# Weepingchestnut/SAVSR

Measured on AMD Instinct MI355X. Metric: HR Mpixels/sec (Vid4-shape x4, 7-frame window), higher is better.
Workload: dtype f32 (bf16x3 split products, fp32 accumulate)

## Files before the change

### savsr_amd/csrc/conv_wy.hip

```cpp
#include "conv_common.hpp"

#include <type_traits>

#ifndef WY_STAMPS
#define WY_STAMPS 0
#endif
#ifndef WY_VALU
#define WY_VALU 6
#endif
#ifndef WY_FAST_EPILOGUE
#define WY_FAST_EPILOGUE 1
#endif
#ifndef WY_BUF
#define WY_BUF 1
#endif

namespace savsr {

namespace wy {
constexpr int TH = 16, TW = 32, NTHR = 512, COT = 64;
[[maybe_unused]] constexpr int IC = TW + 2;
#ifndef WY_ICP
#define WY_ICP 36
#endif
constexpr int ICP = WY_ICP;
constexpr int V_PLANE = 2 * ICP;
constexpr int V_WAVE = 2 * 2 * 2 * V_PLANE;
constexpr int W_HALF = 6 * 2 * 2 * 64;
constexpr int W_PHASE = 2 * W_HALF;
constexpr int EPS = 36;
constexpr int LDS_UNITS = 8 * V_WAVE + 2 * W_HALF;
constexpr size_t LDS_BYTES = 16ull * LDS_UNITS + 4ull * 8 * 32 * EPS;
static_assert(LDS_BYTES <= 160 * 1024, "LDS budget");
}

__device__ __attribute__((aligned(16))) const float g_wy_zero16[4] = {0.f, 0.f, 0.f, 0.f};

#if WY_STAMPS
__device__ long long g_wy_stamps[256 * 8 * 8];
#define WY_KSEC(i) (WY_STAMPS == 2 ? 0 : (i))
#define WY_MARK(i) do { const long long t_now = (long long)__builtin_amdgcn_s_memtime(); wy_sec[i] += t_now - wy_prev; wy_prev = t_now; } while (0)
#if WY_STAMPS == 2
#define WY_EMARK(i) WY_MARK(i)
#endif
#else
#define WY_KSEC(i) (i)
#define WY_MARK(i) do { } while (0)
#endif

__device__ __forceinline__ void wy_split_store(const f32x4& v, bf16x4* hi_dst, bf16x4* lo_dst) {
    bf16x4 hi, lo;
#pragma unroll
    for (int j = 0; j < 4; ++j) {
        const __bf16 hh = (__bf16)v[j];
        hi[j] = hh;
        lo[j] = (__bf16)(v[j] - (float)hh);
    }
    *hi_dst = hi;
    *lo_dst = lo;
}
__device__ __forceinline__ void wy_f16_store(const f32x4& v, bf16x4* hi_dst) {
    f16x4 h;
#pragma unroll
    for (int j = 0; j < 4; ++j) h[j] = (_Float16)v[j];
    *hi_dst = __builtin_bit_cast(bf16x4, h);
}

template <bool FAST, bool F16>
__global__ __launch_bounds__(512) void conv_wy_kernel(const MultiConvParams mp) {
    using namespace wy;
    constexpr int WPH = F16 ? W_PHASE / 2 : W_PHASE, WHF = F16 ? W_HALF / 2 : W_HALF;
    extern __shared__ __attribute__((aligned(16))) unsigned char smem_raw[];
    bf16x8* smem = reinterpret_cast<bf16x8*>(smem_raw);
    const int tid = threadIdx.x, lane = tid & 63, wave = tid >> 6, half = lane >> 5, px = lane & 31;
    const int wave_s = __builtin_amdgcn_readfirstlane(wave);
    const int tiles_per_cob = mp.wy_tiles;
    const int total = mp.nconv * mp.ncob * tiles_per_cob;
    const int H = mp.h, W = mp.w;

    struct TileInfo { int conv, cob, x0, y0, tx, ty, strip; };
    auto decode = [&](int tile) {
        const int cc = (int)((unsigned)tile / (unsigned)tiles_per_cob), rem = tile - cc * tiles_per_cob;
        const bool strip = rem >= mp.wy_full;
        const int tyf = (int)((unsigned)rem / (unsigned)mp.ntx);
        const int l2 = strip ? mp.wy_strip_l2 : 3;
        const int ty = strip ? mp.nty - 1 : tyf;
        const int tx = strip ? (rem - mp.wy_full) << (3 - l2) : rem - tyf * mp.ntx;
        const int wx = tx + (wave_s >> l2);
        TileInfo ti;
        ti.conv = (int)((unsigned)cc / (unsigned)mp.ncob);
        ti.cob = cc - ti.conv * mp.ncob;
        ti.x0 = (wx < mp.ntx ? wx : tx) * TW;
        ti.y0 = wx < mp.ntx ? ty * TH - 2 * ((wave_s >> l2) << l2) : mp.nty * TH;
        ti.tx = tx;
        ti.ty = ty;
        ti.strip = strip ? 1 : 0;
        return ti;
    };

    f32x4 d[2][4], dx;
#if !WY_BUF
    int st_pxb[2], st_pxt;
    constexpr int INVALID = -(1 << 30);
#endif
    const float* st_base = nullptr;
    const bf16x8* st_w = nullptr;
    int st_pix = 0, st_cb = 0, st_src = 0, st_conv = 0, st_row0 = 0;
    const int q4 = lane & 3;
#if WY_BUF
    constexpr unsigned OOB = 0x80000000u;
    unsigned st_vcol[2], st_vtail;
    int st_x0 = 0;
    auto stage_cols = [&]() {
#pragma unroll
        for (int r = 0; r < 2; ++r) {
            const int x = st_x0 - 1 + (lane >> 2) + 16 * r;
            const unsigned v = (unsigned)(x * st_pix + 4 * q4) * 4u;
            st_vcol[r] = (unsigned)x < (unsigned)W ? v : OOB;
        }
        const int x = st_x0 - 1 + 32 + ((lane & 7) >> 2), rr = (lane >> 3) & 3, row = st_row0 + rr;
        const unsigned vt = (unsigned)((rr * W + x) * st_pix + 4 * q4) * 4u;
        const bool okt = (lane < 32) & ((unsigned)x < (unsigned)W) & ((unsigned)row < (unsigned)H);
        st_vtail = okt ? vt : OOB;
    };
#endif
#if WY_BUF
    auto uni = [](int v) { return __builtin_amdgcn_readfirstlane(v); };
    auto uni_ptr = [](const float* q) {
        const unsigned long long a = (unsigned long long)(uintptr_t)q;
        const unsigned lo = (unsigned)__builtin_amdgcn_readfirstlane((int)(unsigned)a), hi = (unsigned)__builtin_amdgcn_readfirstlane((int)(unsigned)(a >> 32));
        return (const float*)(uintptr_t)(((unsigned long long)hi << 32) | lo);
    };
#else
    auto uni = [](int v) { return v; };
    auto uni_ptr = [](const float* q) { return q; };
#endif
    auto stage_begin_tile = [&](const TileInfo& ti) {
        st_conv = ti.conv;
        st_src = 0;
        st_cb = 0;
        st_base = uni_ptr(mp.c[ti.conv].src[0]);
        st_pix = uni(mp.c[ti.conv].src_pix[0]);
        st_w = reinterpret_cast<const bf16x8*>(mp.c[ti.conv].wimg) + (long long)ti.cob * mp.nchunk * WPH;
        st_row0 = uni(ti.y0 + 2 * wave_s - 1);
#if WY_BUF
        st_x0 = ti.x0;
        stage_cols();
#else
#pragma unroll
        for (int r = 0; r < 2; ++r) {
            const int x = ti.x0 - 1 + (lane >> 2) + 16 * r;
            st_pxb[r] = (x >= 0 && x < W) ? st_row0 * W + x : INVALID;
        }
        {
            const int x = ti.x0 - 1 + 32 + ((lane & 7) >> 2), row = st_row0 + ((lane >> 3) & 3);
            st_pxt = (lane < 32 && x >= 0 && x < W && row >= 0 && row < H) ? row * W + x : INVALID;
        }
#endif
    };
    auto stage_advance = [&]() {
        st_cb += 16;
        st_w += WPH;
        if (st_cb >= mp.src_ch) {
            st_cb = 0;
            ++st_src;
            st_base = uni_ptr(mp.c[st_conv].src[st_src]);
#if WY_BUF
            const int pix_new = uni(mp.c[st_conv].src_pix[st_src]);
            if (pix_new != st_pix) { st_pix = pix_new; stage_cols(); }
#else
            st_pix = mp.c[st_conv].src_pix[st_src];
#endif
        }
    };
    int st_tile = blockIdx.x, st_chunk = 0;
    auto stage_next = [&]() -> bool {
        if (st_chunk + 1 < mp.nchunk) { ++st_chunk; stage_advance(); return true; }
        if (st_tile + (int)gridDim.x >= total) return false;
        st_tile += gridDim.x;
        st_chunk = 0;
        stage_begin_tile(decode(st_tile));
        return true;
    };
#if WY_BUF
    typedef unsigned u32x4_t __attribute__((ext_vector_type(4)));
    auto row_rsrc = [&](int i, bool whole) {
        const int off = ((st_row0 + i) * W * st_pix + st_cb) * 4;
        const bool row_ok = whole || (st_row0 + i >= 0 && st_row0 + i < H);
        return __builtin_amdgcn_make_buffer_rsrc((void*)((const char*)st_base + off), (short)0, row_ok ? 0x7fffffff : 0, 0x00020000);
    };
    auto issue_row = [&](int r, int i) {
        d[r][i] = __builtin_bit_cast(f32x4, (u32x4_t)__builtin_amdgcn_raw_buffer_load_b128(row_rsrc(i, false), (int)st_vcol[r], 0, 0));
    };
    auto issue_d = [&](int r) {
#pragma unroll
        for (int i = 0; i < 4; ++i) issue_row(r, i);
    };
    auto issue_dx = [&]() { dx = __builtin_bit_cast(f32x4, (u32x4_t)__builtin_amdgcn_raw_buffer_load_b128(row_rsrc(0, true), (int)st_vtail, 0, 0)); };
#else
    auto load_at = [&](int pixel, bool ok) -> f32x4 {
        const SAVSR_GLOBAL float* src = ok ? (const SAVSR_GLOBAL float*)st_base + (pixel * st_pix + st_cb + 4 * q4)
                                           : (const SAVSR_GLOBAL float*)g_wy_zero16;
        return *(const SAVSR_GLOBAL f32x4*)src;
    };
    auto issue_row = [&](int r, int i) {
        const bool row_ok = st_row0 + i >= 0 && st_row0 + i < H;
        d[r][i] = load_at(st_pxb[r] + i * W, row_ok && st_pxb[r] != INVALID);
    };
    auto issue_d = [&](int r) {
#pragma unroll
        for (int i = 0; i < 4; ++i) issue_row(r, i);
    };
    auto issue_dx = [&]() { dx = load_at(st_pxt, st_pxt != INVALID); };
#endif
    bf16x8* vwave = smem + wave * V_WAVE;
    constexpr int PLANE_B = V_PLANE * 16;
    const unsigned vst0 = (unsigned)(wave * V_WAVE + (q4 >> 1) * ICP + (lane >> 2)) * 16u + (unsigned)(q4 & 1) * 8u;
    const unsigned vst_t = (unsigned)(wave * V_WAVE + (q4 >> 1) * ICP + 32 + ((lane & 7) >> 2)) * 16u + (unsigned)(q4 & 1) * 8u;
    auto vptr = [&](unsigned off) { return reinterpret_cast<bf16x4*>(smem_raw + off); };
    auto vstore = [&](const f32x4& v, unsigned off) {
        if constexpr (F16) wy_f16_store(v, vptr(off));
        else wy_split_store(v, vptr(off), vptr(off + PLANE_B));
    };
    auto store_pair = [&](int r, int hf, const f32x4& va, const f32x4& vb) {
        vstore(va, vst0 + (unsigned)(r * 256 + (hf * 2 + 0) * 2 * PLANE_B));
        vstore(vb, vst0 + (unsigned)(r * 256 + (hf * 2 + 1) * 2 * PLANE_B));
    };
    auto store_one = [&](int r, int hf, int vr, const f32x4& v) {
        vstore(v, vst0 + (unsigned)(r * 256 + (hf * 2 + vr) * 2 * PLANE_B));
    };
    auto store_v0 = [&](int r) { store_one(r, 0, 0, d[r][0] - d[r][2]); };
    auto store_v1 = [&](int r) {
        store_one(r, 0, 1, d[r][1] + d[r][2]);
        const f32x4 v2 = d[r][2] - d[r][1], v3 = d[r][1] - d[r][3];
        d[r][0] = v2;
        d[r][1] = v3;
    };
    auto store_v01 = [&](int r) { store_v0(r); store_v1(r); };
    auto store_v23 = [&](int r) { store_pair(r, 1, d[r][0], d[r][1]); };
    const int grp = (lane >> 3) & 3;
    auto tail_value = [&](int hf) -> f32x4 {
        const int partner = hf == 0 ? (grp == 0 ? lane ^ 16 : lane ^ 24) : (grp == 2 ? lane ^ 24 : lane ^ 16);
        f32x4 o;
#pragma unroll
        for (int j = 0; j < 4; ++j) o[j] = __shfl(dx[j], partner, 64);
        return (hf == 0 && grp == 1) ? dx + o : dx - o;
    };
    auto tail_store = [&](int hf, const f32x4& v) {
        const bool mine = lane < 32 && (hf == 0 ? grp < 2 : (grp == 2 || grp == 1));
        const int vr = hf == 0 ? grp : (grp == 2 ? 0 : 1);
        if (mine) {
            vstore(v, vst_t + (unsigned)((hf * 2 + vr) * 2 * PLANE_B));
        }
    };
    auto store_vt01 = [&]() {
        const f32x4 v01 = tail_value(0), v23 = tail_value(1);
        tail_store(0, v01);
        dx = v23;
    };
    auto store_vt23 = [&]() { tail_store(1, dx); };
    bf16x8* wlds = smem + 8 * V_WAVE;
    [[maybe_unused]] const unsigned lane16 = (unsigned)lane * 16u;
    auto issue_w = [&](int j, int hf) {
        const int piece = F16 ? j * 8 + wave_s : wave_s * 3 + j;
        if (F16 && piece >= 12) return;
        const unsigned dst = __builtin_amdgcn_readfirstlane((unsigned)(uintptr_t)(wlds + hf * W_HALF + piece * (F16 ? 128 : 64)));
        unsigned keep;
#if WY_BUF
        asm volatile("s_mov_b32 %0, m0\n\ts_mov_b32 m0, %3\n\ts_nop 0\n\tglobal_load_lds_dwordx4 %1, %2\n\ts_mov_b32 m0, %0"
                     : "=&s"(keep) : "v"(lane16), "s"(st_w + hf * WHF + piece * 64), "s"(dst) : "memory");
#else
        asm volatile("s_mov_b32 %0, m0\n\ts_mov_b32 m0, %2\n\ts_nop 0\n\tglobal_load_lds_dwordx4 %1, off\n\ts_mov_b32 m0, %0"
                     : "=&s"(keep) : "v"(st_w + hf * WHF + piece * 64 + lane), "s"(dst) : "memory");
#endif
    };

    struct FragA { bf16x8 ah, al; };
    struct FragB { bf16x8 bh, bl; };
    const bf16x8* vrd = vwave + half * ICP + px;
    const bf16x8* wrd = wlds + lane;
    auto load_b = [&](int hf, int s, FragB& fr) {
        const int vr = s / 3, kx = s - 3 * vr;
        fr.bh = vrd[((hf * 2 + vr) * 2 + 0) * V_PLANE + kx];
        if (!F16) fr.bl = vrd[((hf * 2 + vr) * 2 + 1) * V_PLANE + kx];
    };
    auto load_a = [&](int hf, int s, int t, FragA& fr) {
        fr.ah = wrd[hf * W_HALF + ((s * 2 + t) * 2 + 0) * 64];
        if (!F16) fr.al = wrd[hf * W_HALF + ((s * 2 + t) * 2 + 1) * 64];
    };

    int tile = blockIdx.x;
#if WY_STAMPS
    long long wy_sec[8] = {0, 0, 0, 0, 0, 0, 0, 0};
    long long wy_prev = (long long)__builtin_amdgcn_s_memtime();
    const long long wy_t0 = wy_prev;
#endif
    FragA fa[2];
    FragB fb[2];
    if (tile < total) {
        stage_begin_tile(decode(tile));
#pragma unroll
        for (int j = 0; j < 3; ++j) issue_w(j, 0);
        issue_d(0);
        issue_d(1);
        issue_dx();
        store_v01(0);
        store_v01(1);
        store_vt01();
    }
    asm volatile("s_waitcnt vmcnt(0)" ::: "memory");
    __syncthreads();
    if (tile < total) { load_b(0, 0, fb[0]); load_a(0, 0, 0, fa[0]); }

    for (; tile < total; tile += gridDim.x) {
        const TileInfo cur = decode(tile);
        const ConvParams& p = mp.c[cur.conv];
        const int cob = cur.cob, x0 = cur.x0, y0 = cur.y0;
        f32x16 acc[4][2];
#pragma unroll
        for (int pz = 0; pz < 4; ++pz)
#pragma unroll
            for (int t = 0; t < 2; ++t)
#pragma unroll
                for (int i = 0; i < 16; ++i) acc[pz][t][i] = 0.f;
        const bool rows_in = y0 + 2 * wave_s < H;
        for (int chunk = 0; chunk < mp.nchunk; ++chunk) {
            auto phase = [&](auto mm) {
                constexpr bool MM = decltype(mm)::value;
                auto pieces = [&](int hf, int s) {
                    if (hf == 0) {
                        if (s == 0) { issue_w(0, 1); issue_w(1, 1); store_v23(0); }
                        if (s == 1) { issue_w(2, 1); stage_next(); issue_row(0, 0); }
                        if (s == 2) { store_v23(1); issue_row(0, 1); issue_row(0, 2); }
                        if (s == 3) { store_vt23(); issue_row(0, 3); issue_row(1, 0); }
                        if (s == 4) { issue_row(1, 1); issue_row(1, 2); }
                        if (s == 5) issue_row(1, 3);
                    } else {
                        if (s < 3) issue_w(s, 0);
                        if (s == 1) store_v0(0);
                        if (s == 2) store_v1(0);
                        if (s == 3) store_v0(1);
                        if (s == 4) store_v1(1);
                        if (s == 5) store_vt01();
                    }
                };
                auto mma3 = [&](int pz, int t, int sb) {
                    const FragA& a = fa[t];
                    const FragB& b = fb[sb];
                    if (MM && F16) {
                        acc[pz][t] = __builtin_amdgcn_mfma_f32_32x32x16_f16(__builtin_bit_cast(f16x8, a.ah), __builtin_bit_cast(f16x8, b.bh), acc[pz][t], 0, 0, 0);
                    } else if (MM) {
                        acc[pz][t] = __builtin_amdgcn_mfma_f32_32x32x16_bf16(a.al, b.bh, acc[pz][t], 0, 0, 0);
                        acc[pz][t] = __builtin_amdgcn_mfma_f32_32x32x16_bf16(a.ah, b.bl, acc[pz][t], 0, 0, 0);
                        acc[pz][t] = __builtin_amdgcn_mfma_f32_32x32x16_bf16(a.ah, b.bh, acc[pz][t], 0, 0, 0);
                    }
                };
#pragma unroll
                for (int hf = 0; hf < 2; ++hf) {
#pragma unroll
                    for (int s = 0; s < 5; ++s) {
                        const int pz = hf * 2 + s / 3;
                        load_a(hf, s, 1, fa[1]);
                        load_b(hf, s + 1, fb[(s + 1) & 1]);
                        __builtin_amdgcn_sched_barrier(0);
                        mma3(pz, 0, s & 1);
                        pieces(hf, s);
                        load_a(hf, s + 1, 0, fa[0]);
                        mma3(pz, 1, s & 1);
                        if (MM && F16) {
#pragma unroll
                            for (int i = 0; i < 2; ++i) {
                                __builtin_amdgcn_sched_group_barrier(0x008, 1, 0);
                                if (i == 1) __builtin_amdgcn_sched_group_barrier(0x100, 1, 0);
                                __builtin_amdgcn_sched_group_barrier(0x002, 3 * WY_VALU, 0);
                                __builtin_amdgcn_sched_group_barrier(0x200, 2, 0);
                                __builtin_amdgcn_sched_group_barrier(0x010, 1, 0);
                            }
                        } else if (MM) {
#pragma unroll
                            for (int i = 0; i < 6; ++i) {
                                __builtin_amdgcn_sched_group_barrier(0x008, 1, 0);
                                if (i == 3) __builtin_amdgcn_sched_group_barrier(0x100, 2, 0);
                                __builtin_amdgcn_sched_group_barrier(0x002, WY_VALU, 0);
                                __builtin_amdgcn_sched_group_barrier(0x200, 1, 0);
                                if (i == 1 || i == 4) __builtin_amdgcn_sched_group_barrier(0x010, 1, 0);
                            }
                        }
                        __builtin_amdgcn_sched_barrier(0);
                    }
                    {
                        const int pz = hf * 2 + 1;
                        load_a(hf, 5, 1, fa[1]);
                        __builtin_amdgcn_sched_barrier(0);
                        mma3(pz, 0, 1);
                        pieces(hf, 5);
                        if (MM) {
#pragma unroll
                            for (int i = 0; i < (F16 ? 1 : 3); ++i) {
                                __builtin_amdgcn_sched_group_barrier(0x008, 1, 0);
                                __builtin_amdgcn_sched_group_barrier(0x002, 10, 0);
                                __builtin_amdgcn_sched_group_barrier(0x200, 1, 0);
                            }
                        }
                        __builtin_amdgcn_sched_barrier(0);
                        WY_MARK(WY_KSEC(hf * 3 + 0));
                        if (hf == 0) asm volatile("s_waitcnt vmcnt(8)" ::: "memory");
                        else asm volatile("s_waitcnt vmcnt(0)" ::: "memory");
                        __syncthreads();
                        WY_MARK(WY_KSEC(hf * 3 + 1));
                        load_b(hf ^ 1, 0, fb[0]);
                        load_a(hf ^ 1, 0, 0, fa[0]);
                        __builtin_amdgcn_sched_barrier(0);
                        mma3(pz, 1, 1);
                        if (hf == 0) issue_dx();
                        __builtin_amdgcn_sched_barrier(0);
                    }
                    WY_MARK(WY_KSEC(hf * 3 + 2));
                }
            };
            if (rows_in) phase(std::true_type{}); else phase(std::false_type{});
        }

        const float* e_bias = p.bias;
        const float* e_mul = p.mul_px;
        const float* e_r1 = p.res1;
        const float* e_r2 = p.res2;
        float* e_out = p.out;
        float* e_pool = p.pool;
        int e_act = p.act, e_opix = p.out_pix, e_r1pix = p.res1_pix, e_r2pix = p.res2_pix;
        float e_slope = p.slope, e_r2s = p.res2_scale;
        asm volatile("" : "+s"(e_bias), "+s"(e_mul), "+s"(e_r1), "+s"(e_r2), "+s"(e_out), "+s"(e_pool));
        asm volatile("" : "+s"(e_act), "+s"(e_opix), "+s"(e_r1pix), "+s"(e_r2pix), "+s"(e_slope), "+s"(e_r2s));
        const bool act_as_max = e_act == SAVSR_ACT_NONE || e_act == SAVSR_ACT_RELU || (e_act == SAVSR_ACT_LRELU && e_slope >= 0.f && e_slope <= 1.f);
        const float slope_eff = e_act == SAVSR_ACT_NONE ? 1.f : (e_act == SAVSR_ACT_RELU ? 0.f : e_slope);
        float* ep_base = reinterpret_cast<float*>(smem + LDS_UNITS);
        float* ep = ep_base + wave * (32 * EPS);
        const int c4 = lane & 7;
        const bool x_inside = x0 + TW <= W;
        const float* zero16 = (const float*)g_wy_zero16;
        const float* b_base = e_bias ? e_bias : zero16;
        const unsigned b_off = e_bias ? 4u * (unsigned)(cob * COT + 4 * c4) : 0u, b_step = e_bias ? 128u : 0u;
        f32x4 bias4[2];
#pragma unroll
        for (int t = 0; t < 2; ++t) bias4[t] = ldg4(b_base, b_off + (unsigned)t * b_step);
        const float* r1_base = e_r1 ? e_r1 : zero16;
        constexpr int RR = 2;
        f32x4 rr[RR][4];
        auto load_r1 = [&](int r, int t, f32x4 (&dst)[4]) {
            const int y = y0 + 2 * wave_s + r;
            const int co = cob * COT + 32 * t + 4 * c4;
            const unsigned off0 = 4u * (unsigned)((y * W + x0 + (lane >> 3)) * e_r1pix + co), ustride = 32u * (unsigned)e_r1pix;
            const bool row_ok = e_r1 && y < H;
#pragma unroll
            for (int i = 0; i < 4; ++i) {
                const bool ok = row_ok && (x_inside || x0 + (lane >> 3) + 8 * i < W);
                dst[i] = ldg4(r1_base, ok ? off0 + (unsigned)i * ustride : 0u);
            }
        };
#pragma unroll
        for (int gi = 0; gi < RR; ++gi) load_r1(gi / 2, gi % 2, rr[gi]);
        __builtin_amdgcn_sched_barrier(0);
#pragma unroll
        for (int t = 0; t < 2; ++t)
#pragma unroll
            for (int i = 0; i < 16; ++i) {
                const float m1 = acc[1][t][i], m2 = acc[2][t][i];
                acc[0][t][i] = (acc[0][t][i] + m1) + m2;
                acc[3][t][i] = (m1 - m2) - acc[3][t][i];
            }
        f32x4 psum[2][2];
#ifdef WY_EMARK
        asm volatile("" :: "v"(acc[0][0][0]), "v"(acc[3][1][15]));
        WY_EMARK(1);
#endif
#pragma unroll
        for (int r = 0; r < 2; ++r) {
            const int y = y0 + 2 * wave_s + r;
            const int pbase = y * W + x0 + (lane >> 3);
#pragma unroll
            for (int t = 0; t < 2; ++t) {
                psum[r][t] = f32x4{0.f, 0.f, 0.f, 0.f};
                const int gi = r * 2 + t;
                if (y >= H) {
                    asm volatile("" :: "v"(bias4[t]), "v"(rr[gi % RR][0]), "v"(rr[gi % RR][1]), "v"(rr[gi % RR][2]), "v"(rr[gi % RR][3]));
                    if (gi + RR < 4) load_r1((gi + RR) / 2, (gi + RR) % 2, rr[gi % RR]);
                    continue;
                }
                const f32x16& a = r == 0 ? acc[0][t] : acc[3][t];
#pragma unroll
                for (int g = 0; g < 4; ++g) {
                    const f32x4 v = {a[4 * g], a[4 * g + 1], a[4 * g + 2], a[4 * g + 3]};
                    *reinterpret_cast<f32x4*>(ep + px * EPS + 8 * g + 4 * half) = v;
                }
                const int co = cob * COT + 32 * t + 4 * c4;
                const f32x4 b4 = bias4[t];
                const unsigned ooff0 = 4u * (unsigned)(pbase * e_opix + co), ostride = 32u * (unsigned)e_opix;
                f32x4 ps = {0.f, 0.f, 0.f, 0.f};
#pragma unroll
                for (int ih = 0; ih < 2; ++ih) {
                    const int p0 = pbase + 16 * ih;
                    const bool ok0 = x_inside || x0 + (lane >> 3) + 16 * ih < W, ok1 = x_inside || x0 + (lane >> 3) + 16 * ih + 8 < W;
                    f32x4 v[2];
#pragma unroll
                    for (int i = 0; i < 2; ++i) {
                        const f32x4 a4 = *reinterpret_cast<const f32x4*>(ep + ((lane >> 3) + 16 * ih + 8 * i) * EPS + 4 * c4);
                        v[i] = a4 + b4;
                    }
                    if constexpr (FAST) {
#pragma unroll
                        for (int i = 0; i < 2; ++i) {
                            const f32x4 sv = v[i] * slope_eff;
#pragma unroll
                            for (int q = 0; q < 4; ++q) v[i][q] = vmax_raw(v[i][q], sv[q]);
                        }
                    } else if (e_act == SAVSR_ACT_NONE) {
                    } else if (act_as_max) {
#pragma unroll
                        for (int i = 0; i < 2; ++i) {
                            const f32x4 sv = v[i] * slope_eff;
#pragma unroll
                            for (int q = 0; q < 4; ++q) v[i][q] = vmax_raw(v[i][q], sv[q]);
                        }
                    } else if (e_act == SAVSR_ACT_LRELU) {
#pragma unroll
                        for (int i = 0; i < 2; ++i)
#pragma unroll
                            for (int q = 0; q < 4; ++q) v[i][q] = v[i][q] > 0.f ? v[i][q] : v[i][q] * e_slope;
                    } else if (e_act == SAVSR_ACT_SIGMOID) {
#pragma unroll
                        for (int i = 0; i < 2; ++i)
#pragma unroll
                            for (int q = 0; q < 4; ++q) v[i][q] = sigmoidf_(v[i][q]);
                    }
                    if (!FAST && e_mul) {
                        const float m0 = ok0 ? ldg1(e_mul, (unsigned)p0) : 0.f, m1 = ok1 ? ldg1(e_mul, (unsigned)(p0 + 8)) : 0.f;
#pragma unroll
                        for (int q = 0; q < 4; ++q) { v[0][q] *= m0; v[1][q] *= m1; }
                    }
                    v[0] += rr[gi % RR][2 * ih];
                    v[1] += rr[gi % RR][2 * ih + 1];
                    if (!FAST && e_r2) {
                        f32x4 ra = {0.f, 0.f, 0.f, 0.f}, rb = {0.f, 0.f, 0.f, 0.f};
                        if (ok0) ra = ldg4(e_r2, 4u * (unsigned)(p0 * e_r2pix + co));
                        if (ok1) rb = ldg4(e_r2, 4u * (unsigned)((p0 + 8) * e_r2pix + co));
#pragma unroll
                        for (int q = 0; q < 4; ++q) { v[0][q] += e_r2s * ra[q]; v[1][q] += e_r2s * rb[q]; }
                    }
#pragma unroll
                    for (int i = 0; i < 2; ++i) {
                        if (i == 0 ? ok0 : ok1) {
                            stg4(e_out, ooff0 + (unsigned)(2 * ih + i) * ostride, v[i]);
                            if (e_pool) ps += v[i];
                        }
                    }
                }
                psum[r][t] = ps;
#ifdef WY_EMARK
                WY_EMARK(2 + gi);
#endif
                if (gi + RR < 4) load_r1((gi + RR) / 2, (gi + RR) % 2, rr[gi % RR]);
            }
        }
        if (e_pool) {
#pragma unroll
            for (int r = 0; r < 2; ++r)
#pragma unroll
                for (int t = 0; t < 2; ++t)
#pragma unroll
                    for (int o = 8; o < 64; o <<= 1) {
                        psum[r][t][0] += __shfl_xor(psum[r][t][0], o, 64); psum[r][t][1] += __shfl_xor(psum[r][t][1], o, 64);
                        psum[r][t][2] += __shfl_xor(psum[r][t][2], o, 64); psum[r][t][3] += __shfl_xor(psum[r][t][3], o, 64);
                    }
            __syncthreads();
            float* pl_ = ep_base;
            if (lane < 8)
#pragma unroll
                for (int r = 0; r < 2; ++r)
#pragma unroll
                    for (int t = 0; t < 2; ++t) *reinterpret_cast<f32x4*>(pl_ + (wave * 2 + r) * COT + 32 * t + 4 * lane) = psum[r][t];
            __syncthreads();
            const TileInfo pt = decode(tile);
            const int l2p = pt.strip ? mp.wy_strip_l2 : 2;
            if (tid < (8 >> l2p) * COT) {
                const int sg = tid / COT, ch = tid - sg * COT;
                float sacc = 0.f;
#pragma unroll
                for (int k = 0; k < 8; ++k)
                    if (k < (2 << l2p)) sacc += pl_[(((sg << l2p) * 2) + k) * COT + ch];
                const int band = pt.ty * 2 + (pt.strip ? 0 : sg), ptx = pt.tx + (pt.strip ? sg : 0);
                if (band * 8 < H && ptx < mp.ntx) stg1(e_pool, (unsigned)((band * mp.ntx + ptx) * p.pool_stride + cob * COT + ch), sacc);
            }
            __syncthreads();
        }
        WY_MARK(6);
    }
#if WY_STAMPS
    wy_sec[7] = (long long)__builtin_amdgcn_s_memtime() - wy_t0;
    if (lane == 0 && blockIdx.x < 256)
        for (int i = 0; i < 8; ++i) g_wy_stamps[(blockIdx.x * 8 + wave) * 8 + i] = wy_sec[i];
#endif
    asm volatile("s_waitcnt vmcnt(0)" ::: "memory");
}

int launch_conv_wy(const MultiConvParams& mp, hipStream_t st, bool f16) {
    if (int rc = conv_wy_prepare_device()) return rc;
    const int total = mp.nconv * mp.ncob * mp.wy_tiles;
    const int grid = total < CONV_PERSISTENT_BLOCKS ? total : CONV_PERSISTENT_BLOCKS;
    bool fast = WY_FAST_EPILOGUE != 0;
    for (int i = 0; i < mp.nconv && fast; ++i) {
        const ConvParams& c = mp.c[i];
        const bool as_max = c.act == SAVSR_ACT_NONE || c.act == SAVSR_ACT_RELU || (c.act == SAVSR_ACT_LRELU && c.slope >= 0.f && c.slope <= 1.f);
        fast = as_max && !c.mul_px && !c.res2;
    }
    if (f16) {
        if (fast) hipLaunchKernelGGL((conv_wy_kernel<true, true>), dim3(grid), dim3(wy::NTHR), wy::LDS_BYTES, st, mp);
        else hipLaunchKernelGGL((conv_wy_kernel<false, true>), dim3(grid), dim3(wy::NTHR), wy::LDS_BYTES, st, mp);
    } else if (fast) hipLaunchKernelGGL((conv_wy_kernel<true, false>), dim3(grid), dim3(wy::NTHR), wy::LDS_BYTES, st, mp);
    else hipLaunchKernelGGL((conv_wy_kernel<false, false>), dim3(grid), dim3(wy::NTHR), wy::LDS_BYTES, st, mp);
    return check_launch("conv_wy_kernel");
}
int conv_wy_prepare_device() {
    if (int rc = ensure_dynamic_lds(reinterpret_cast<const void*>(&conv_wy_kernel<true, false>), (int)wy::LDS_BYTES, "conv_wy")) return rc;
    if (int rc = ensure_dynamic_lds(reinterpret_cast<const void*>(&conv_wy_kernel<false, false>), (int)wy::LDS_BYTES, "conv_wy")) return rc;
    if (int rc = ensure_dynamic_lds(reinterpret_cast<const void*>(&conv_wy_kernel<true, true>), (int)wy::LDS_BYTES, "conv_wy")) return rc;
    return ensure_dynamic_lds(reinterpret_cast<const void*>(&conv_wy_kernel<false, true>), (int)wy::LDS_BYTES, "conv_wy");
}

}

using namespace savsr;

#if WY_STAMPS
extern "C" int savsr_debug_read_wy_stamps(long long* host) {
    return (int)hipMemcpyFromSymbol(host, HIP_SYMBOL(g_wy_stamps), sizeof(long long) * 256 * 8 * 8);
}
#endif

extern "C" int64_t savsr_conv_wy_packed_elems(int cout, int cin) {
    if (cout <= 0 || cout % 64 || cin <= 0 || cin % 16) return -1;
    return (int64_t)(cout / 64) * (cin / 16) * 12 * 16 * 64;
}
extern "C" int64_t savsr_conv_wy_pack_index(int cout, int cin, int co, int ci, int pos, int kx) {
    const int64_t nchunk = cin / 16;
    const int cob = co / 64, col = co % 64, t = col / 32, row = col % 32;
    const int chunk = ci / 16, cl = ci % 16, kh = cl / 8, j = cl % 8;
    const int hf = pos / 2, vr = pos % 2, s = vr * 3 + kx;
    const int64_t group = ((((int64_t)(cob * nchunk + chunk) * 2 + hf) * 6 + s) * 2 + t);
    return group * 512 + (kh * 32 + row) * 8 + j;
}
```

Measured before the change: 142.1.

## Skip MMA work for out-of-range row waves and pack bf16 split conversion

Waves whose rows fall entirely below the image bottom now run a reduced 'dead' phase. It only issues weight loads, stages the next chunk and keeps the barrier cadence, instead of running the full MMA pipeline on padding. On the last chunk the full phase still runs when the next tile's rows are in range, presumably to preserve cross-tile prefetch. Separately, the hi/lo bf16 split now uses packed two-wide conversions and recovers the hi part with bit shifts, to cut VALU instructions. The dead path must keep the same barrier count and loads as the full phase, or the kernel risks deadlock or stale data.

```diff
diff --git a/savsr_amd/csrc/conv_wy.hip b/savsr_amd/csrc/conv_wy.hip
--- a/savsr_amd/csrc/conv_wy.hip
+++ b/savsr_amd/csrc/conv_wy.hip
@@ -48,16 +48,23 @@
 #define WY_MARK(i) do { } while (0)
 #endif
 
+typedef float f32x2 __attribute__((ext_vector_type(2)));
+typedef __bf16 bf16x2 __attribute__((ext_vector_type(2)));
 __device__ __forceinline__ void wy_split_store(const f32x4& v, bf16x4* hi_dst, bf16x4* lo_dst) {
-    bf16x4 hi, lo;
-#pragma unroll
-    for (int j = 0; j < 4; ++j) {
-        const __bf16 hh = (__bf16)v[j];
-        hi[j] = hh;
-        lo[j] = (__bf16)(v[j] - (float)hh);
+    typedef unsigned u32x2 __attribute__((ext_vector_type(2)));
+    const f32x2 a[2] = {{v[0], v[1]}, {v[2], v[3]}};
+    u32x2 hi, lo;
+#pragma unroll
+    for (int p = 0; p < 2; ++p) hi[p] = __builtin_bit_cast(unsigned, __builtin_convertvector(a[p], bf16x2));
+    asm("" : "+v"(hi[0]), "+v"(hi[1]));
+#pragma unroll
+    for (int p = 0; p < 2; ++p) {
+        const f32x2 back = {__builtin_bit_cast(float, hi[p] << 16), __builtin_bit_cast(float, hi[p] & 0xffff0000u)};
+        const f32x2 rest = {a[p][0] - back[0], a[p][1] - back[1]};
+        lo[p] = __builtin_bit_cast(unsigned, __builtin_convertvector(rest, bf16x2));
     }
-    *hi_dst = hi;
-    *lo_dst = lo;
+    *hi_dst = __builtin_bit_cast(bf16x4, hi);
+    *lo_dst = __builtin_bit_cast(bf16x4, lo);
 }
 __device__ __forceinline__ void wy_f16_store(const f32x4& v, bf16x4* hi_dst) {
     f16x4 h;
@@ -418,7 +425,24 @@
                     WY_MARK(WY_KSEC(hf * 3 + 2));
                 }
             };
-            if (rows_in) phase(std::true_type{}); else phase(std::false_type{});
+            auto phase_dead = [&]() {
+#pragma unroll
+                for (int j = 0; j < 3; ++j) issue_w(j, 1);
+                stage_next();
+                asm volatile("s_waitcnt vmcnt(0)" ::: "memory");
+                __syncthreads();
+#pragma unroll
+                for (int j = 0; j < 3; ++j) issue_w(j, 0);
+                asm volatile("s_waitcnt vmcnt(0)" ::: "memory");
+                __syncthreads();
+            };
+            auto next_tile_rows_in = [&]() {
+                if (tile + (int)gridDim.x >= total) return false;
+                return decode(tile + (int)gridDim.x).y0 + 2 * wave_s < H;
+            };
+            if (rows_in) phase(std::true_type{});
+            else if (chunk + 1 == mp.nchunk && next_tile_rows_in()) phase(std::false_type{});
+            else phase_dead();
         }
 
         const float* e_bias = p.bias;
```

Result: faster. 144.2 (median of 6 runs) (+1.4%).
